# febrianrachmadi/dep-gan-im

Hardware: AMD Instinct MI355X
Metric: 2D slices/sec (G+2D+GP train step), 256x256x1 fp32 (higher is better)
Workload: dtype f32; 1 GPU; DEP-GAN-IM twoCritics canonical train step (critic-Y2 + critic-DEM + G update, WGAN-GP), batch 32 per GPU, 256x256x1; per_gpu_batch=32, global_batch=32, parallelism=dp1

## Files before the change

dep_gan_im_amd/csrc/igemm_wino.hip:

```cpp
#include <stdlib.h>

#include <type_traits>

#include "common.h"
#include "epilogue.h"

namespace {

constexpr int WN_CK = 8;
constexpr int WN_TW = 18;
constexpr int WN_CP = 36;
constexpr int WN_XV = WN_CK / 4;

template <int MT>
struct WnCfg {
  static constexpr int TH = 8 * MT;
  static constexpr int NTILE = 32 * MT;
  static constexpr int PIXT = (TH + 2) * WN_TW;
  static constexpr int XTOT = PIXT * WN_XV;
  static constexpr int NXP = (XTOT + 255) / 256;
  static constexpr int RAW = NXP * 256 * 4;
  static_assert(XTOT % 4 == 0 && WN_TW % 2 == 0, "rslot permutes inside aligned groups of four slots: halo and padding stay apart");
  static constexpr int ZPLANE = NTILE * WN_CP + 32;
  static constexpr int Z = 8 * ZPLANE;
  static constexpr int NBUF = 2;
  static_assert(NBUF >= 2 && NBUF * RAW <= Z, "the raw ring must fit under the Z exchange: LDS and workgroups per CU unchanged");
  static_assert((NBUF - 1) * NXP + 4 < 64, "counted waits: vmcnt is a 6-bit field");
  static constexpr size_t LDS = sizeof(float) * (size_t)Z;
  static constexpr int WGS_PER_CU = (MT == 2) ? 2 : 3;
};

template <int N>
static __device__ __forceinline__ void wn_wait_vm() {
  asm volatile("s_waitcnt vmcnt(%0)" ::"n"(N) : "memory");
}
template <int NX, int Y>
static __device__ __forceinline__ void wn_wait_younger(int y) {
  if constexpr (Y == 0) {
    wn_wait_vm<4>();
  } else {
    if (y >= Y) wn_wait_vm<NX * Y + 4>();
    else wn_wait_younger<NX, Y - 1>(y);
  }
}

static __device__ __forceinline__ int rslot(int pix, int half) { return (2 * pix + half) ^ (((pix % WN_TW) >> 2) & 3); }
static __device__ __forceinline__ int rslot_inv(int q) { return q ^ ((((q >> 1) % WN_TW) >> 2) & 3); }

template <int MT, bool PERS, bool HEAD, int ABL = 0>
static __device__ __forceinline__ void wino_body(const ConvArgs& a) {
  typedef WnCfg<MT> C;
  constexpr int MF = 32, NT = 32;
  constexpr int WN_RAW = C::RAW, WN_ZPLANE = C::ZPLANE, WN_XTOT = C::XTOT, NXP = C::NXP, NBUF = C::NBUF;
  constexpr int NXI = (ABL & 8) ? 0 : NXP;
  typedef f32x16 acc_t;
  extern __shared__ __attribute__((aligned(16))) float smem[];

  const int tid = threadIdx.x;
  const int lane = tid & 63, wv = tid >> 6;
  const int r = lane & 31, h = lane >> 5;
  const int tilesX = (a.W + 15) >> 4, tilesY = (a.H + C::TH - 1) / C::TH;
  const unsigned nNTall = (unsigned)a.lgy, nPix = (unsigned)a.lgx;
  const int nCC = a.Cin / WN_CK;

  constexpr int SENT = (int)0x80000000;
  int xvo[NXP], xyx[NXP];
#pragma unroll
  for (int i = 0; i < NXP; ++i) {
    const int q = tid + i * 256;
    const int lq = rslot_inv(q);
    const int pix = lq >> 1, part = lq & 1;
    const int ly = pix / WN_TW, lx = pix - ly * WN_TW;
    xvo[i] = (q < WN_XTOT) ? 4 * (ly * (int)a.in.sY + lx * (int)a.in.sX + part * 4) : SENT;
    xyx[i] = (ly << 8) | lx;
  }
  int tA[MT][4], tB[MT][4];
  float tS[MT];
#pragma unroll
  for (int i = 0; i < MT; ++i) {
    const int cg = h, aa = wv, T = 32 * i + r;
    const int tyi = T >> 3, txi = T & 7;
    const int rA = (aa == 0) ? 0 : (aa == 2 ? 2 : 1), rB = (aa == 3) ? 3 : (aa == 2 ? 1 : 2);
#pragma unroll
    for (int j = 0; j < 4; ++j) {
      tA[i][j] = 16 * rslot((2 * tyi + rA) * WN_TW + 2 * txi + j, cg);
      tB[i][j] = 16 * rslot((2 * tyi + rB) * WN_TW + 2 * txi + j, cg);
    }
    tS[i] = (aa == 1) ? 1.f : -1.f;
  }
  const int wbase = __builtin_amdgcn_readfirstlane(wv * 256);
  const int boff = (4 * wv * 32 + r) * WN_CK + 4 * h;

  unsigned id = blockIdx.x;
  do {
    int t, ntile;
    if ((nPix & 7u) == 0) {
      const unsigned x = id & 7u, sl = id >> 3;
      ntile = (int)(sl % nNTall);
      t = (int)(x * (nPix >> 3) + sl / nNTall);
    } else {
      t = (int)(id % nPix);
      ntile = (int)(id / nPix);
    }
    const int tx0 = (t % tilesX) * 16;
    t /= tilesX;
    const int ty0 = (t % tilesY) * C::TH;
    const int b = t / tilesY;
    const long out_goff = 0;
    const int n0 = ntile * NT;
    const float* inb = a.in.p + (long)b * a.in.sB;
    const bool interior = ty0 >= 1 && ty0 + C::TH + 1 <= a.H && tx0 >= 1 && tx0 + 17 <= a.W;
    const char* halo0 = reinterpret_cast<const char*>(inb + ((long)(ty0 - 1) * a.in.sY + (long)(tx0 - 1) * a.in.sX));
    auto coff = [&](int cc) -> long {
      if (a.cpt > 0) {
        const int run = cc / a.cpt;
        return a.in_run_off[run] + (long)(cc - run * a.cpt) * WN_CK;
      }
      return (long)cc * WN_CK;
    };
    const float* const xorg = a.in.p - ((long)a.in.sY + (long)a.in.sX);
    const unsigned long long xu = (unsigned long long)xorg;
    const unsigned xlo = __builtin_amdgcn_readfirstlane((unsigned)xu), xhi = __builtin_amdgcn_readfirstlane((unsigned)(xu >> 32));
    const __amdgpu_buffer_rsrc_t rx =
        __builtin_amdgcn_make_buffer_rsrc((void*)(((unsigned long long)xhi << 32) | xlo), 0, 0x7FFFFFFF, 0x00020000);
    const int xso0 = 4 * (b * (int)a.in.sB + ty0 * (int)a.in.sY + tx0 * (int)a.in.sX);
    auto stage_dma = [&](int cc, int buf) {
      const int xso = xso0 + 4 * (int)coff(cc);
      float* xs = smem + buf * WN_RAW + wbase;
      if (interior) {
#pragma unroll
        for (int i = 0; i < NXP; ++i) {
          const int vo = xvo[i];
          __builtin_amdgcn_raw_ptr_buffer_load_lds(rx, (__attribute__((address_space(3))) void*)(xs + i * 1024), 16, vo,
                                                   xso, 0, 0);
        }
      } else {
#pragma unroll
        for (int i = 0; i < NXP; ++i) {
          const int iy = ty0 + (xyx[i] >> 8) - 1, ix = tx0 + (xyx[i] & 255) - 1;
          const int vo = (iy >= 0 && iy < a.H && ix >= 0 && ix < a.W) ? xvo[i] : SENT;
          __builtin_amdgcn_raw_ptr_buffer_load_lds(rx, (__attribute__((address_space(3))) void*)(xs + i * 1024), 16, vo,
                                                   xso, 0, 0);
        }
      }
    };

    acc_t acc[4][MT];

    const float* wnt = a.w + (size_t)ntile * nCC * (16 * NT * WN_CK) + boff;
    if (!(ABL & 8)) {
#pragma unroll
      for (int k = 0; k < NBUF - 1; ++k)
        if (k < nCC) stage_dma(k, k);
    }
    auto chunk = [&](const int cc, const int slot, auto first_tag) {
      constexpr bool FIRST = decltype(first_tag)::value;
      const bool issue = cc + NBUF - 1 < nCC;
      f32x4 bq[4];
      {
        const float* wp = wnt + (size_t)cc * (16 * NT * WN_CK);
        static_assert(3 * NT * WN_CK * sizeof(float) < 4096, "immediate offsets of the fragment loads");
        asm volatile(
            "global_load_dwordx4 %0, %4, off\n\t"
            "global_load_dwordx4 %1, %4, off offset:1024\n\t"
            "global_load_dwordx4 %2, %4, off offset:2048\n\t"
            "global_load_dwordx4 %3, %4, off offset:3072"
            : "=&v"(bq[0]), "=&v"(bq[1]), "=&v"(bq[2]), "=&v"(bq[3])
            : "v"(wp)
            : "memory");
        static_assert(NT * WN_CK * sizeof(float) == 1024, "the offsets above");
      }
      wn_wait_younger<NXI, NBUF - 2>(nCC - 1 - cc);
      __builtin_amdgcn_s_barrier();
      asm volatile("" ::: "memory");
      if (issue && !(ABL & 8)) stage_dma(cc + NBUF - 1, slot ? slot - 1 : NBUF - 1);
      const char* raw = reinterpret_cast<const char*>(smem + slot * WN_RAW);
      f32x2 vr[MT][4][2];
      if (ABL & 2) {
#pragma unroll
        for (int i = 0; i < MT; ++i)
#pragma unroll
          for (int bb = 0; bb < 4; ++bb) vr[i][bb][0] = vr[i][bb][1] = f32x2{0.f, 0.f};
      }
#pragma unroll
      for (int i = 0; i < ((ABL & 2) ? 0 : MT); ++i) {
        const f32x2 s2 = {tS[i], tS[i]};
        f32x2 tc[4][2];
        f32x4 xs[4], ys[4];
#pragma unroll
        for (int j = 0; j < 4; ++j) {
          xs[j] = *reinterpret_cast<const f32x4*>(raw + tA[i][j]);
          ys[j] = *reinterpret_cast<const f32x4*>(raw + tB[i][j]);
        }
        __builtin_amdgcn_sched_barrier(0);
#pragma unroll
        for (int j = 0; j < 4; ++j) {
          const f32x4 x = xs[j], y = ys[j];
          tc[j][0] = __builtin_elementwise_fma(f32x2{y[0], y[1]}, s2, f32x2{x[0], x[1]});
          tc[j][1] = __builtin_elementwise_fma(f32x2{y[2], y[3]}, s2, f32x2{x[2], x[3]});
        }
#pragma unroll
        for (int p = 0; p < 2; ++p) {
          vr[i][0][p] = tc[0][p] - tc[2][p];
          vr[i][1][p] = tc[1][p] + tc[2][p];
          vr[i][2][p] = tc[2][p] - tc[1][p];
          vr[i][3][p] = tc[1][p] - tc[3][p];
        }
      }
#pragma unroll
      for (int i = 0; i < MT; ++i)
        asm volatile("" : "+v"(vr[i][0][0]), "+v"(vr[i][0][1]), "+v"(vr[i][1][0]), "+v"(vr[i][1][1]), "+v"(vr[i][2][0]),
                          "+v"(vr[i][2][1]), "+v"(vr[i][3][0]), "+v"(vr[i][3][1]));
      __builtin_amdgcn_sched_barrier(0);
      if (issue) wn_wait_vm<NXI>();
      else wn_wait_vm<0>();
      asm volatile("" : "+v"(bq[0]), "+v"(bq[1]), "+v"(bq[2]), "+v"(bq[3])::"memory");
#pragma unroll
      for (int f = 0; f < 4; ++f) {
        __builtin_amdgcn_sched_barrier(0);
#pragma unroll
        for (int j = 0; j < 4; ++j)
#pragma unroll
          for (int mt = 0; mt < MT; ++mt)
            if (!(ABL & 4)) {
              if (FIRST && j == 0) {
                const acc_t zero = {0.f, 0.f, 0.f, 0.f, 0.f, 0.f, 0.f, 0.f, 0.f, 0.f, 0.f, 0.f, 0.f, 0.f, 0.f, 0.f};
                acc[f][mt] = __builtin_amdgcn_mfma_f32_32x32x2f32(bq[f][j], vr[mt][f][j >> 1][j & 1], zero, 0, 0, 0);
              } else {
                acc[f][mt] = __builtin_amdgcn_mfma_f32_32x32x2f32(bq[f][j], vr[mt][f][j >> 1][j & 1], acc[f][mt], 0, 0, 0);
              }
            } else {
              if (FIRST && j == 0) acc[f][mt] = acc_t{};
              acc[f][mt][j] += bq[f][j] * vr[mt][f][j >> 1][j & 1];
            }
        __builtin_amdgcn_sched_barrier(0);
      }
    };
    chunk(0, 0, std::true_type{});
    for (int cc = 1, s = 1 % NBUF; cc < nCC; ++cc, s = (s + 1 == NBUF) ? 0 : s + 1) chunk(cc, s, std::false_type{});

    if (ABL & 1) {
      float sacc = 0.f;
#pragma unroll
      for (int f = 0; f < 4; ++f)
#pragma unroll
        for (int mt = 0; mt < MT; ++mt)
#pragma unroll
          for (int j = 0; j < 16; ++j) sacc += acc[f][mt][j];
      if (sacc == 12345.678f) a.out.p[tid] = sacc;
      __syncthreads();
      continue;
    }
    auto zstage = [&]() {
      __syncthreads();
      float* zw = smem + (2 * wv) * WN_ZPLANE + r * WN_CP + 4 * h;
#pragma unroll
      for (int mt = 0; mt < MT; ++mt)
#pragma unroll
        for (int g = 0; g < 4; ++g) {
          f32x4 z0, z1;
#pragma unroll
          for (int k = 0; k < 4; ++k) {
            const float m0 = acc[0][mt][4 * g + k], m1 = acc[1][mt][4 * g + k], m2 = acc[2][mt][4 * g + k],
                        m3 = acc[3][mt][4 * g + k];
            z0[k] = (m0 + m1) + m2;
            z1[k] = (m1 - m2) - m3;
          }
          *reinterpret_cast<f32x4*>(zw + mt * (32 * WN_CP) + 8 * g) = z0;
          *reinterpret_cast<f32x4*>(zw + WN_ZPLANE + mt * (32 * WN_CP) + 8 * g) = z1;
        }
      __syncthreads();
    };
#define EPI_PRE_SYNC
#define EPI_STAGE
#define EPI_STAGE_LATE zstage()
#define EPI_NPASS (4 * MT)
#define EPI_OYW (ty0 + 2 * MT * __builtin_amdgcn_readfirstlane(wv))
#define EPI_FULL ((ty0 + C::TH <= a.H) && (tx0 + 16 <= a.W))
#define EPI_FETCH(v, py, px)                                                                                         \
  {                                                                                                                  \
    const float* zb = smem + ((px)&1) * WN_ZPLANE +                                                                  \
                      ((MT * __builtin_amdgcn_readfirstlane(wv) + ((py) >> 1)) * 8 + ((px) >> 1)) * WN_CP + c4;       \
    const f32x4 za = *reinterpret_cast<const f32x4*>(zb + (((py)&1) ? 2 : 0) * WN_ZPLANE);                           \
    const f32x4 zb1 = *reinterpret_cast<const f32x4*>(zb + (((py)&1) ? 4 : 2) * WN_ZPLANE);                          \
    const f32x4 zc = *reinterpret_cast<const f32x4*>(zb + (((py)&1) ? 6 : 4) * WN_ZPLANE);                           \
    _Pragma("unroll") for (int k_ = 0; k_ < 4; ++k_) v[k_] = ((py)&1) ? (za[k_] - zb1[k_]) - zc[k_] : (za[k_] + zb1[k_]) + zc[k_]; \
  }
#define EPI_HEAD HEAD
#include "igemm_epilogue.inc"
#undef EPI_HEAD
#undef EPI_FETCH
#undef EPI_FULL
#undef EPI_OYW
#undef EPI_NPASS
#undef EPI_STAGE_LATE
#undef EPI_STAGE
#undef EPI_PRE_SYNC
    if (PERS) __syncthreads();
  } while (PERS && (id += gridDim.x) < nPix * nNTall);
}

template <int MT, bool PERS>
__global__ __launch_bounds__(256, WnCfg<MT>::WGS_PER_CU) void wino_conv_kernel(const ConvArgs a) {
  wino_body<MT, PERS, false>(a);
}
template <bool PERS>
__global__ __launch_bounds__(256, 2) void wino_conv_head_kernel(const ConvArgs a) {
  wino_body<2, PERS, true>(a);
}
#ifdef DEPGAN_WINO_ABLATIONS
template <int MT, int ABL>
__global__ __launch_bounds__(256, WnCfg<MT>::WGS_PER_CU) void wino_conv_abl_kernel(const ConvArgs a) {
  wino_body<MT, true, false, ABL>(a);
}
#endif

}

bool dg_conv_wino_supported(const ConvPlan& pl, const ConvArgs& a) {
  if (!dg_plan_wino(pl)) return false;
  if (a.Cin != pl.Cin || (a.Cin % WN_CK) || (a.Cout % 32) || a.groups > 1 || a.dbg || ((a.H | a.W) & 1)) return false;
  if (a.cpt > 0 && ((a.Cin % (a.cpt * WN_CK)) != 0 || a.Cin / (a.cpt * WN_CK) > 4)) return false;
  return true;
}

static int wino_mt(const ConvArgs& a) {
  static int forced = -1;
  if (forced < 0) {
    const char* e = getenv("DEPGAN_WINO_MT");
    forced = e ? atoi(e) : 0;
  }
  if (a.ep.head_out) return 2;
  if (forced == 1 || forced == 2) return forced;
  return 1;
}

template <int MT>
static void wino_geometry(ConvArgs& a, long* total, long* G, bool* pers) {
  a.lgx = cdiv(a.W, 16) * cdiv(a.H, WnCfg<MT>::TH) * a.B;
  a.lgy = a.Cout / 32;
  *total = (long)a.lgx * a.lgy;
  const long cap = (long)WnCfg<MT>::WGS_PER_CU * dg_cu_count();
  *pers = *total > cap;
  *G = *pers ? cap : *total;
}

const char* dg_conv_wino_name(const ConvArgs& a_in) {
  ConvArgs a = a_in;
  long total, G;
  bool pers;
  const int mt = wino_mt(a);
  if (mt == 2) wino_geometry<2>(a, &total, &G, &pers); else wino_geometry<1>(a, &total, &G, &pers);
  if (a.ep.head_out) return pers ? "wino_conv_head_kernel<true>" : "wino_conv_head_kernel<false>";
  if (mt == 2) return pers ? "wino_conv_kernel<2,true>" : "wino_conv_kernel<2,false>";
  return pers ? "wino_conv_kernel<1,true>" : "wino_conv_kernel<1,false>";
}

template <int MT>
static int wino_launch(ConvArgs a, hipStream_t st) {
  long total, G;
  bool pers;
  wino_geometry<MT>(a, &total, &G, &pers);
  constexpr size_t LDS = WnCfg<MT>::LDS;
  static DgOncePerDevice once;
  if (once.need()) {
    HIPCHECK(hipFuncSetAttribute(reinterpret_cast<const void*>(&wino_conv_kernel<MT, false>),
                                 hipFuncAttributeMaxDynamicSharedMemorySize, (int)LDS));
    HIPCHECK(hipFuncSetAttribute(reinterpret_cast<const void*>(&wino_conv_kernel<MT, true>),
                                 hipFuncAttributeMaxDynamicSharedMemorySize, (int)LDS));
    if (MT == 2) {
      HIPCHECK(hipFuncSetAttribute(reinterpret_cast<const void*>(&wino_conv_head_kernel<false>),
                                   hipFuncAttributeMaxDynamicSharedMemorySize, (int)LDS));
      HIPCHECK(hipFuncSetAttribute(reinterpret_cast<const void*>(&wino_conv_head_kernel<true>),
                                   hipFuncAttributeMaxDynamicSharedMemorySize, (int)LDS));
    }
  }
#ifdef DEPGAN_WINO_ABLATIONS
  if (const char* e = getenv("DEPGAN_WINO_ABL")) {
    const int abl = atoi(e);
    if (abl && pers && !a.ep.head_out) {
#define WN_ABL_CASE(N)                                                                                              \
  case N:                                                                                                           \
    HIPCHECK(hipFuncSetAttribute(reinterpret_cast<const void*>(&wino_conv_abl_kernel<MT, N>),                       \
                                 hipFuncAttributeMaxDynamicSharedMemorySize, (int)LDS));                            \
    hipLaunchKernelGGL((wino_conv_abl_kernel<MT, N>), dim3((unsigned)G), dim3(256), LDS, st, a);                    \
    break;
      switch (abl) {
        WN_ABL_CASE(1) WN_ABL_CASE(2) WN_ABL_CASE(3) WN_ABL_CASE(4) WN_ABL_CASE(8) WN_ABL_CASE(10) WN_ABL_CASE(11)
        default: dg_set_error("DEPGAN_WINO_ABL=%d not instantiated", abl); return DG_ERR_ARG;
      }
      HIPCHECK(hipGetLastError());
      return DG_OK;
    }
  }
#endif
  if (a.ep.head_out) {
    if (MT != 2 || a.Cout != 32 || a.ep.pool.p) {
      dg_set_error("dg_conv_wino: the fused head needs 32 output channels and no fused pool");
      return DG_ERR_ARG;
    }
    if (pers) hipLaunchKernelGGL((wino_conv_head_kernel<true>), dim3((unsigned)G), dim3(256), LDS, st, a);
    else hipLaunchKernelGGL((wino_conv_head_kernel<false>), dim3((unsigned)G), dim3(256), LDS, st, a);
  } else {
    if (pers) hipLaunchKernelGGL((wino_conv_kernel<MT, true>), dim3((unsigned)G), dim3(256), LDS, st, a);
    else hipLaunchKernelGGL((wino_conv_kernel<MT, false>), dim3((unsigned)G), dim3(256), LDS, st, a);
  }
  HIPCHECK(hipGetLastError());
  return DG_OK;
}

int dg_conv_wino(const ConvPlan& pl, const ConvArgs& a, hipStream_t st) {
  if (!dg_conv_wino_supported(pl, a)) {
    dg_set_error("dg_conv_wino: shape not covered (3x3, Cin %% 8, Cout %% 32, even H and W, no groups)");
    return DG_ERR_UNSUPPORTED;
  }
  return wino_mt(a) == 2 ? wino_launch<2>(a, st) : wino_launch<1>(a, st);
}
```

Measured before the change: 667.4 slices/s.

## Prefetch next persistent work item's first input chunk across item boundary in Winograd conv

For the MT=1 persistent Winograd kernel, adds an extra LDS raw buffer beyond the Z exchange region and stages the first channel chunk of the next work item during the last chunk (or the epilogue) of the current one. The ring logic becomes a fixed two-slot alternation and the trailing per-item __syncthreads is dropped, with explicit barriers and lgkmcnt waits around the Z staging. The aim is to hide the DMA latency at the start of each persistent item. It costs more LDS per workgroup, though a static assert keeps occupancy unchanged, and the barrier and wait logic becomes more fragile.

After: 673.3 slices/s, median of 6. Within noise of the previous version (+0.9%).

```diff
diff --git a/dep_gan_im_amd/csrc/igemm_wino.hip b/dep_gan_im_amd/csrc/igemm_wino.hip
--- a/dep_gan_im_amd/csrc/igemm_wino.hip
+++ b/dep_gan_im_amd/csrc/igemm_wino.hip
@@ -28,6 +28,10 @@
   static_assert((NBUF - 1) * NXP + 4 < 64, "counted waits: vmcnt is a 6-bit field");
   static constexpr size_t LDS = sizeof(float) * (size_t)Z;
   static constexpr int WGS_PER_CU = (MT == 2) ? 2 : 3;
+  static constexpr bool XITEM = (MT == 1);
+  static constexpr size_t LDS_PERS = LDS + (XITEM ? sizeof(float) * (size_t)RAW : 0);
+  static_assert(WGS_PER_CU * LDS_PERS <= 160 * 1024, "the prefetch buffer must not cost a workgroup per CU");
+  static_assert(!XITEM || (NBUF == 2 && LDS_PERS == 46080), "cross-item prefetch: written for a ring of two under Z");
 };
 
 template <int N>
@@ -47,7 +51,11 @@
 static __device__ __forceinline__ int rslot(int pix, int half) { return (2 * pix + half) ^ (((pix % WN_TW) >> 2) & 3); }
 static __device__ __forceinline__ int rslot_inv(int q) { return q ^ ((((q >> 1) % WN_TW) >> 2) & 3); }
 
-template <int MT, bool PERS, bool HEAD, int ABL = 0>
+struct WnItem {
+  int ntile, b, ty0, tx0, xso0;
+  bool interior;
+};
+template <int MT, bool PERS, bool HEAD, int ABL = 0, bool XI = (PERS && !HEAD && WnCfg<MT>::XITEM)>
 static __device__ __forceinline__ void wino_body(const ConvArgs& a) {
   typedef WnCfg<MT> C;
   constexpr int MF = 32, NT = 32;
@@ -91,39 +99,98 @@
   const int wbase = __builtin_amdgcn_readfirstlane(wv * 256);
   const int boff = (4 * wv * 32 + r) * WN_CK + 4 * h;
 
-  unsigned id = blockIdx.x;
-  do {
-    int t, ntile;
+  auto coff = [&](int cc) -> long {
+    if (a.cpt > 0) {
+      const int run = cc / a.cpt;
+      return a.in_run_off[run] + (long)(cc - run * a.cpt) * WN_CK;
+    }
+    return (long)cc * WN_CK;
+  };
+  const int coff0 = XI ? 4 * (int)coff(0) : 0;
+  auto decode = [&](unsigned id_) -> WnItem {
+    WnItem it;
+    int t;
     if ((nPix & 7u) == 0) {
-      const unsigned x = id & 7u, sl = id >> 3;
-      ntile = (int)(sl % nNTall);
+      const unsigned x = id_ & 7u, sl = id_ >> 3;
+      it.ntile = (int)(sl % nNTall);
       t = (int)(x * (nPix >> 3) + sl / nNTall);
     } else {
-      t = (int)(id % nPix);
-      ntile = (int)(id / nPix);
-    }
-    const int tx0 = (t % tilesX) * 16;
+      t = (int)(id_ % nPix);
+      it.ntile = (int)(id_ / nPix);
+    }
+    it.tx0 = (t % tilesX) * 16;
     t /= tilesX;
-    const int ty0 = (t % tilesY) * C::TH;
-    const int b = t / tilesY;
+    it.ty0 = (t % tilesY) * C::TH;
+    it.b = t / tilesY;
+    return it;
+  };
+  auto is_interior = [&](const WnItem& it) {
+    return it.ty0 >= 1 && it.ty0 + C::TH + 1 <= a.H && it.tx0 >= 1 && it.tx0 + 17 <= a.W;
+  };
+  auto halo_off = [&](const WnItem& it) {
+    return 4 * (it.b * (int)a.in.sB + it.ty0 * (int)a.in.sY + it.tx0 * (int)a.in.sX);
+  };
+  auto decode_all = [&](unsigned id_) -> WnItem {
+    WnItem it = decode(id_);
+    it.interior = is_interior(it);
+    it.xso0 = halo_off(it) + coff0;
+    return it;
+  };
+  auto mkrx = [&]() {
+    const float* const xorg = a.in.p - ((long)a.in.sY + (long)a.in.sX);
+    const unsigned long long xu = (unsigned long long)xorg;
+    const unsigned xlo = __builtin_amdgcn_readfirstlane((unsigned)xu), xhi = __builtin_amdgcn_readfirstlane((unsigned)(xu >> 32));
+    return __builtin_amdgcn_make_buffer_rsrc((void*)(((unsigned long long)xhi << 32) | xlo), 0, 0x7FFFFFFF, 0x00020000);
+  };
+  auto stage_first = [&](const __amdgpu_buffer_rsrc_t rx, const WnItem& it) {
+    const int ty0 = it.ty0, tx0 = it.tx0, xso = it.xso0;
+    const bool interior = it.interior;
+    float* xs = smem + C::Z + wbase;
+    if (interior) {
+#pragma unroll
+      for (int i = 0; i < NXP; ++i) {
+        const int vo = xvo[i];
+        __builtin_amdgcn_raw_ptr_buffer_load_lds(rx, (__attribute__((address_space(3))) void*)(xs + i * 1024), 16, vo,
+                                                 xso, 0, 0);
+      }
+    } else {
+#pragma unroll
+      for (int i = 0; i < NXP; ++i) {
+        const int iy = ty0 + (xyx[i] >> 8) - 1, ix = tx0 + (xyx[i] & 255) - 1;
+        const int vo = (iy >= 0 && iy < a.H && ix >= 0 && ix < a.W) ? xvo[i] : SENT;
+        __builtin_amdgcn_raw_ptr_buffer_load_lds(rx, (__attribute__((address_space(3))) void*)(xs + i * 1024), 16, vo,
+                                                 xso, 0, 0);
+      }
+    }
+  };
+
+  unsigned id = blockIdx.x;
+  WnItem nx;
+  if (XI) {
+    nx = decode_all(id);
+    const __amdgpu_buffer_rsrc_t rx = mkrx();
+    if (!(ABL & 8)) stage_first(rx, nx);
+  }
+  do {
+    WnItem it;
+    bool more = false;
+    if (XI) {
+      it = nx;
+      const unsigned idn = id + gridDim.x;
+      more = idn < nPix * nNTall;
+      if (more) nx = decode_all(idn);
+    } else {
+      it = decode(id);
+    }
+    const int ntile = it.ntile, b = it.b, ty0 = it.ty0, tx0 = it.tx0;
     const long out_goff = 0;
     const int n0 = ntile * NT;
     const float* inb = a.in.p + (long)b * a.in.sB;
-    const bool interior = ty0 >= 1 && ty0 + C::TH + 1 <= a.H && tx0 >= 1 && tx0 + 17 <= a.W;
+    const bool interior = XI ? it.interior : is_interior(it);
     const char* halo0 = reinterpret_cast<const char*>(inb + ((long)(ty0 - 1) * a.in.sY + (long)(tx0 - 1) * a.in.sX));
-    auto coff = [&](int cc) -> long {
-      if (a.cpt > 0) {
-        const int run = cc / a.cpt;
-        return a.in_run_off[run] + (long)(cc - run * a.cpt) * WN_CK;
-      }
-      return (long)cc * WN_CK;
-    };
-    const float* const xorg = a.in.p - ((long)a.in.sY + (long)a.in.sX);
-    const unsigned long long xu = (unsigned long long)xorg;
-    const unsigned xlo = __builtin_amdgcn_readfirstlane((unsigned)xu), xhi = __builtin_amdgcn_readfirstlane((unsigned)(xu >> 32));
-    const __amdgpu_buffer_rsrc_t rx =
-        __builtin_amdgcn_make_buffer_rsrc((void*)(((unsigned long long)xhi << 32) | xlo), 0, 0x7FFFFFFF, 0x00020000);
-    const int xso0 = 4 * (b * (int)a.in.sB + ty0 * (int)a.in.sY + tx0 * (int)a.in.sX);
+    const __amdgpu_buffer_rsrc_t rx = mkrx();
+    const int xso0 = XI ? it.xso0 - coff0 : halo_off(it);
+    const bool prefetch = XI && more && !(ABL & 24);
     auto stage_dma = [&](int cc, int buf) {
       const int xso = xso0 + 4 * (int)coff(cc);
       float* xs = smem + buf * WN_RAW + wbase;
@@ -148,14 +215,16 @@
     acc_t acc[4][MT];
 
     const float* wnt = a.w + (size_t)ntile * nCC * (16 * NT * WN_CK) + boff;
-    if (!(ABL & 8)) {
+    if (!XI && !(ABL & 8) && !((ABL & 16) && id != blockIdx.x)) {
 #pragma unroll
       for (int k = 0; k < NBUF - 1; ++k)
         if (k < nCC) stage_dma(k, k);
     }
     auto chunk = [&](const int cc, const int slot, auto first_tag) {
       constexpr bool FIRST = decltype(first_tag)::value;
-      const bool issue = cc + NBUF - 1 < nCC;
+      const bool ring = cc + NBUF - 1 < nCC;
+      const bool pref = XI && !FIRST && prefetch && cc == nCC - 1;
+      const bool issue = ring || pref;
       f32x4 bq[4];
       {
         const float* wp = wnt + (size_t)cc * (16 * NT * WN_CK);
@@ -173,8 +242,13 @@
       wn_wait_younger<NXI, NBUF - 2>(nCC - 1 - cc);
       __builtin_amdgcn_s_barrier();
       asm volatile("" ::: "memory");
-      if (issue && !(ABL & 8)) stage_dma(cc + NBUF - 1, slot ? slot - 1 : NBUF - 1);
-      const char* raw = reinterpret_cast<const char*>(smem + slot * WN_RAW);
+      if (XI) {
+        if (ring && !(ABL & 8)) stage_dma(cc + 1, slot);
+        if (pref) stage_first(rx, nx);
+      } else {
+        if (issue && !(ABL & 8)) stage_dma(cc + NBUF - 1, slot ? slot - 1 : NBUF - 1);
+      }
+      const char* raw = reinterpret_cast<const char*>((XI && FIRST) ? smem + C::Z : smem + (XI ? 1 - slot : slot) * WN_RAW);
       f32x2 vr[MT][4][2];
       if (ABL & 2) {
 #pragma unroll
@@ -237,7 +311,11 @@
       }
     };
     chunk(0, 0, std::true_type{});
-    for (int cc = 1, s = 1 % NBUF; cc < nCC; ++cc, s = (s + 1 == NBUF) ? 0 : s + 1) chunk(cc, s, std::false_type{});
+    if (XI) {
+      for (int cc = 1, s = 1; cc < nCC; ++cc, s = 1 - s) chunk(cc, s, std::false_type{});
+    } else {
+      for (int cc = 1, s = 1 % NBUF; cc < nCC; ++cc, s = (s + 1 == NBUF) ? 0 : s + 1) chunk(cc, s, std::false_type{});
+    }
 
     if (ABL & 1) {
       float sacc = 0.f;
@@ -249,10 +327,17 @@
           for (int j = 0; j < 16; ++j) sacc += acc[f][mt][j];
       if (sacc == 12345.678f) a.out.p[tid] = sacc;
       __syncthreads();
+      if (XI && prefetch && nCC == 1) stage_first(rx, nx);
       continue;
     }
     auto zstage = [&]() {
-      __syncthreads();
+      if (XI) {
+        __builtin_amdgcn_s_barrier();
+        asm volatile("" ::: "memory");
+        if (prefetch && nCC == 1) stage_first(rx, nx);
+      } else {
+        __syncthreads();
+      }
       float* zw = smem + (2 * wv) * WN_ZPLANE + r * WN_CP + 4 * h;
 #pragma unroll
       for (int mt = 0; mt < MT; ++mt)
@@ -269,7 +354,13 @@
           *reinterpret_cast<f32x4*>(zw + mt * (32 * WN_CP) + 8 * g) = z0;
           *reinterpret_cast<f32x4*>(zw + WN_ZPLANE + mt * (32 * WN_CP) + 8 * g) = z1;
         }
-      __syncthreads();
+      if (XI) {
+        asm volatile("s_waitcnt lgkmcnt(0)" ::: "memory");
+        __builtin_amdgcn_s_barrier();
+        asm volatile("" ::: "memory");
+      } else {
+        __syncthreads();
+      }
     };
 #define EPI_PRE_SYNC
 #define EPI_STAGE
@@ -296,7 +387,7 @@
 #undef EPI_STAGE_LATE
 #undef EPI_STAGE
 #undef EPI_PRE_SYNC
-    if (PERS) __syncthreads();
+    if (PERS && !XI) __syncthreads();
   } while (PERS && (id += gridDim.x) < nPix * nNTall);
 }
 
@@ -361,13 +452,13 @@
   long total, G;
   bool pers;
   wino_geometry<MT>(a, &total, &G, &pers);
-  constexpr size_t LDS = WnCfg<MT>::LDS;
+  constexpr size_t LDS = WnCfg<MT>::LDS, LDSP = WnCfg<MT>::LDS_PERS;
   static DgOncePerDevice once;
   if (once.need()) {
     HIPCHECK(hipFuncSetAttribute(reinterpret_cast<const void*>(&wino_conv_kernel<MT, false>),
                                  hipFuncAttributeMaxDynamicSharedMemorySize, (int)LDS));
     HIPCHECK(hipFuncSetAttribute(reinterpret_cast<const void*>(&wino_conv_kernel<MT, true>),
-                                 hipFuncAttributeMaxDynamicSharedMemorySize, (int)LDS));
+                                 hipFuncAttributeMaxDynamicSharedMemorySize, (int)LDSP));
     if (MT == 2) {
       HIPCHECK(hipFuncSetAttribute(reinterpret_cast<const void*>(&wino_conv_head_kernel<false>),
                                    hipFuncAttributeMaxDynamicSharedMemorySize, (int)LDS));
@@ -382,11 +473,11 @@
 #define WN_ABL_CASE(N)                                                                                              \
   case N:                                                                                                           \
     HIPCHECK(hipFuncSetAttribute(reinterpret_cast<const void*>(&wino_conv_abl_kernel<MT, N>),                       \
-                                 hipFuncAttributeMaxDynamicSharedMemorySize, (int)LDS));                            \
-    hipLaunchKernelGGL((wino_conv_abl_kernel<MT, N>), dim3((unsigned)G), dim3(256), LDS, st, a);                    \
+                                 hipFuncAttributeMaxDynamicSharedMemorySize, (int)LDSP));                           \
+    hipLaunchKernelGGL((wino_conv_abl_kernel<MT, N>), dim3((unsigned)G), dim3(256), LDSP, st, a);                   \
     break;
       switch (abl) {
-        WN_ABL_CASE(1) WN_ABL_CASE(2) WN_ABL_CASE(3) WN_ABL_CASE(4) WN_ABL_CASE(8) WN_ABL_CASE(10) WN_ABL_CASE(11)
+        WN_ABL_CASE(1) WN_ABL_CASE(2) WN_ABL_CASE(3) WN_ABL_CASE(4) WN_ABL_CASE(8) WN_ABL_CASE(10) WN_ABL_CASE(11) WN_ABL_CASE(16)
         default: dg_set_error("DEPGAN_WINO_ABL=%d not instantiated", abl); return DG_ERR_ARG;
       }
       HIPCHECK(hipGetLastError());
@@ -402,7 +493,7 @@
     if (pers) hipLaunchKernelGGL((wino_conv_head_kernel<true>), dim3((unsigned)G), dim3(256), LDS, st, a);
     else hipLaunchKernelGGL((wino_conv_head_kernel<false>), dim3((unsigned)G), dim3(256), LDS, st, a);
   } else {
-    if (pers) hipLaunchKernelGGL((wino_conv_kernel<MT, true>), dim3((unsigned)G), dim3(256), LDS, st, a);
+    if (pers) hipLaunchKernelGGL((wino_conv_kernel<MT, true>), dim3((unsigned)G), dim3(256), LDSP, st, a);
     else hipLaunchKernelGGL((wino_conv_kernel<MT, false>), dim3((unsigned)G), dim3(256), LDS, st, a);
   }
   HIPCHECK(hipGetLastError());
```
